# CDCgov/zoe

Measured on AMD Instinct MI355X. Metric: read-alignments/sec (150 bp vs 2 kb ref), higher is better.
Workload: dtype int16

## Files before the change

### include/zoe_sw.h

```cpp
#ifndef ZOE_SW_H
#define ZOE_SW_H

#include <stddef.h>
#include <stdint.h>

#ifdef __cplusplus
extern "C" {
#endif

typedef enum zsw_error {
    ZSW_OK = 0,
    ZSW_ERR_EMPTY_SEQUENCE = 1,
    ZSW_ERR_GAP_OPEN_OUT_OF_RANGE = 2,
    ZSW_ERR_GAP_EXTEND_OUT_OF_RANGE = 3,
    ZSW_ERR_BAD_GAP_WEIGHTS = 4,
    ZSW_ERR_INVALID_ARGUMENT = -1,
    ZSW_ERR_HIP = -2,
    ZSW_ERR_NO_DEVICE = -3,
    ZSW_ERR_UNSUPPORTED = -4,
    ZSW_ERR_NOT_CONFIGURED = -5
} zsw_error;

typedef enum zsw_status {
    ZSW_STATUS_SOME = 0,
// ... 291 lines not shown
    ZSW_DEBUG_NO_PIPELINE = 32,
    ZSW_DEBUG_ALIGN_NO_PACKED = 64,
    ZSW_DEBUG_SCORE_PRUNE = 128,
    ZSW_DEBUG_SCORE_PRUNE_ANY_SIZE = 256,
    ZSW_DEBUG_PRUNE_STRIP = 512,
    ZSW_DEBUG_ALIGN_LONG_WARMUP = 1024,
    ZSW_DEBUG_SEED_NO_BAND = 2048,
    ZSW_DEBUG_SEED_WIDE_BAND = 4096,
    ZSW_DEBUG_NO_ROW_CHUNKS = 8192,
    ZSW_DEBUG_RANGES_EXACT_REVERSE = 16384,
    ZSW_DEBUG_ALIGN_NO_CERTIFICATE = 32768,
    ZSW_DEBUG_SEED_STRIP_FIRST_TIER = 65536,
    ZSW_DEBUG_SEED_DIAG_LANE_EVENTS = 131072,
    ZSW_DEBUG_SEED_NO_COSCHEDULE = 262144,
    ZSW_DEBUG_SEED_PLAIN_KERNEL = 524288,
    ZSW_DEBUG_SEED_DIAG_MASKED = 1048576
} zsw_debug_flag;
zsw_error zsw_debug_set(zsw_context* ctx, uint32_t flags);

zsw_error zsw_debug_band_records(zsw_context* ctx, int32_t* records);

zsw_error zsw_debug_cert_records(zsw_context* ctx, int32_t* records);

zsw_error zsw_debug_threepass_records(zsw_context* ctx, int32_t* records);

zsw_error zsw_debug_strand_records(zsw_context* ctx, int32_t* records);

zsw_error zsw_debug_panel_records(zsw_context* ctx, int32_t* records);

typedef enum zsw_launch_kind {
    ZSW_LAUNCH_V1_FAST = 0,
// ... 25 lines not shown
```

### zoe_amd/_lib.py

```python
from __future__ import annotations

import ctypes as C
import os

_HERE = os.path.dirname(os.path.abspath(__file__))
LIB_PATH = os.path.join(_HERE, "libzoe_sw_hip.so")

ZSW_OK = 0
ERROR_NAMES = {
    0: "ZSW_OK",
    1: "ProfileError::EmptySequence",
    2: "ProfileError::GapOpenOutOfRange",
    3: "ProfileError::GapExtendOutOfRange",
    4: "ProfileError::BadGapWeights",
    -1: "ZSW_ERR_INVALID_ARGUMENT",
    -2: "ZSW_ERR_HIP",
    -3: "ZSW_ERR_NO_DEVICE",
    -4: "ZSW_ERR_UNSUPPORTED",
    -5: "ZSW_ERR_NOT_CONFIGURED",
}
MEM_HOST, MEM_DEVICE = 0, 1
DEBUG_SCORE_V1, DEBUG_NO_TILES, DEBUG_NO_W32, DEBUG_NO_WIDE, DEBUG_NO_SIDE_STREAMS, DEBUG_NO_PIPELINE, DEBUG_ALIGN_NO_PACKED = 1, 2, 4, 8, 16, 32, 64
DEBUG_SCORE_PRUNE, DEBUG_SCORE_PRUNE_ANY_SIZE, DEBUG_PRUNE_STRIP, DEBUG_ALIGN_LONG_WARMUP, DEBUG_SEED_NO_BAND, DEBUG_SEED_WIDE_BAND = 128, 256, 512, 1024, 2048, 4096
DEBUG_NO_ROW_CHUNKS = 8192
DEBUG_RANGES_EXACT_REVERSE = 16384
DEBUG_ALIGN_NO_CERTIFICATE = 32768
DEBUG_SEED_STRIP_FIRST_TIER = 65536
DEBUG_SEED_DIAG_LANE_EVENTS = 131072
DEBUG_SEED_NO_COSCHEDULE = 262144
DEBUG_SEED_PLAIN_KERNEL = 524288
DEBUG_SEED_DIAG_MASKED = 1048576
(LAUNCH_V1_FAST, LAUNCH_V1_BIASED, LAUNCH_V2, LAUNCH_WIDE, LAUNCH_V1_FAST_REV, LAUNCH_V1_BIASED_REV, LAUNCH_WIDE_REV, LAUNCH_TILE_V2, LAUNCH_TILE_WIDE,
 LAUNCH_TILE_W32, LAUNCH_EXACT32, LAUNCH_EXACT32_WORKLIST, LAUNCH_SEED_WINDOW, LAUNCH_SEED_BAND, LAUNCH_PRUNED, LAUNCH_ROW_CHUNKS) = range(16)
OPTION_EXACT_PRUNING = 1
OPTION_MIN_SCORE = 2
INT_TYPES = {"i8": 0, "i16": 1, "i32": 2, "u8": 3, "u16": 4, "u32": 5}

SYMBOLS = [
    "zsw_pack4_host", "zsw_create", "zsw_destroy", "zsw_last_error_string", "zsw_device_count", "zsw_set_scoring", "zsw_set_reference",
    "zsw_score_batch", "zsw_score_batch_from", "zsw_score_ends_batch", "zsw_score_ranges_batch", "zsw_score_ranges_batch_from", "zsw_align_batch", "zsw_align_batch_from", "zsw_align_3pass_batch", "zsw_align_3pass_batch_from", "zsw_sneaky_snake_batch",
    "zsw_set_profile_sequence", "zsw_score_shared_batch", "zsw_score_shared_batch_from", "zsw_score_ends_shared_batch", "zsw_score_ranges_shared_batch",
    "zsw_score_ranges_shared_batch_from", "zsw_align_shared_batch", "zsw_align_shared_batch_from", "zsw_align_3pass_shared_batch", "zsw_align_3pass_shared_batch_from",
    "zsw_synth_reads", "zsw_synth_reads_ragged", "zsw_synth_length", "zsw_synth_reference_host", "zsw_synth_reads_host",
    "zsw_synth_reads_ragged_host", "zsw_selftest", "zsw_timing_enable", "zsw_timing_read", "zsw_timing_read_window", "zsw_debug_set", "zsw_debug_band_records", "zsw_debug_cert_records", "zsw_debug_threepass_records", "zsw_prune_rescored", "zsw_set_option",
    "zsw_group_create", "zsw_group_destroy", "zsw_group_size", "zsw_group_context", "zsw_group_last_error_string", "zsw_group_set_scoring",
    "zsw_group_set_reference", "zsw_group_score_batch_from", "zsw_group_score_batch_from_device", "zsw_group_align_batch_from",
# ... 212 lines not shown
```

### zoe_amd/build.py

```python
from __future__ import annotations

import os
import shutil
import subprocess
import sys

HERE = os.path.dirname(os.path.abspath(__file__))
CSRC = os.path.join(HERE, "csrc")
LIB = os.path.join(HERE, "libzoe_sw_hip.so")
SOURCES = ["zsw_capi.hip", "zsw_capi_shared.hip", "zsw_shared.hip", "zsw_score.hip", "zsw_align.hip", "zsw_align_pk8.hip", "zsw_align_pk16.hip", "zsw_align_pk32.hip", "zsw_align_pk64.hip", "zsw_group.hip", "zsw_threepass.hip", "zsw_filter.hip", "zsw_score_wide.hip", "zsw_score_w32.hip", "zsw_score_prune.hip", "zsw_score_seed.hip", "zsw_score_seed_m0.hip", "zsw_score_seed_m1.hip", "zsw_score_seed_m2.hip", "zsw_score_band.hip", "zsw_multi.hip", "zsw_strand.hip", "zsw_panel.hip", "zsw_annotate.hip", "zsw_sam.hip", "zsw_pileup.hip", "zsw_text.hip", "zsw_fastq.hip", "zsw_samtext.hip", "zsw_fasta.hip"]
HEADERS = ["zsw_internal.hpp", "zsw_align_dev.hpp", "zsw_align_pk.hpp", "zsw_align_pk_kernel.hpp", "zsw_score_v1.hpp", "zsw_score_v2.hpp", "zsw_handback.hpp", "zsw_score_prune.hpp", "zsw_seed.hpp", "zsw_seed_packed.hpp", "zsw_seed_diag.hpp", "zsw_seed_diag_body.inc", "zsw_cert.hpp", "zsw_context.hpp", "zsw_shared.hpp", "zsw_score_seed.hpp", "zsw_score_seed_kernel.hpp", "zsw_align.hpp", "zsw_timer.hpp", "zsw_strand.hpp", "zsw_panel.hpp", "zsw_annotate.hpp", "zsw_sam.hpp", "zsw_pileup.hpp", "zsw_wave.hpp", "zsw_text.hpp", "zsw_text_dev.hpp", "zsw_fastq.hpp", "zsw_samtext.hpp", "zsw_fasta.hpp", "zsw_synth.h", "zsw_exports.map", os.path.join("..", "..", "include", "zoe_sw.h")]
ARCH = "gfx950"
EXTRA_FLAGS = {}


def _hipcc() -> str:
    for cand in (shutil.which("hipcc"), "/opt/rocm/bin/hipcc"):
        if cand and os.path.exists(cand):
            return cand
    raise RuntimeError("hipcc not found: the HIP extension cannot be built")


def needs_build() -> bool:
    if not os.path.exists(LIB):
        return True
# ... 75 lines not shown
```

### zoe_amd/csrc/zsw_capi.hip

```cpp
#include <map>
#include <new>
#include <utility>

#include "zsw_context.hpp"
#include "zsw_cert.hpp"
#include "zsw_strand.hpp"
#include "zsw_synth.h"

using namespace zsw;
using namespace zsw::capi;

namespace zsw {
namespace capi {


__global__ void maxlen_kernel(const uint64_t* offsets, uint32_t n, uint32_t* out) {
    uint32_t i = blockIdx.x * blockDim.x + threadIdx.x;
    uint32_t m = 0;
    for (; i < n; i += gridDim.x * blockDim.x) m = max(m, (uint32_t)(offsets[i + 1] - offsets[i]));
    for (int d = 32; d >= 1; d >>= 1) m = max(m, (uint32_t)__shfl_xor((int)m, d, 64));
    if ((threadIdx.x & 63) == 0) atomicMax(out, m);
}

__global__ void synth_kernel(uint64_t seed, uint64_t first, uint64_t n, uint32_t len, const uint8_t* ref, uint32_t R,
// ... 113 lines not shown
                           reads->offsets, n, ctx->d_maxlen.as<uint32_t>());
        uint32_t m = 0;
        ZSW_HIP(ctx, hipMemcpyAsync(&m, ctx->d_maxlen.p, 4, hipMemcpyDeviceToHost, stream));
        ZSW_HIP(ctx, hipStreamSynchronize(stream));
        st->max_len = m;
    }
    if (dest) st->dev = *dest;
    return ZSW_OK;
}

static zsw_error common_score_workspace(zsw_context* ctx, const Against& t, const zsw_batch* reads, hipStream_t stream, Staged* st) {
    const uint32_t n = st->b.n_reads;
    ZSW_HIP(ctx, ctx->d_fb_list.ensure((size_t)n * 4 + 4));
    ZSW_HIP(ctx, ctx->d_fb_count.ensure(4));
    if (reads->offsets || st->max_len > LONGEST_STRIP) ZSW_HIP(ctx, ctx->d_bucket_items.ensure((size_t)n * 4 + 4));
    if (reads->offsets && !ctx->side) {
        SideStreams* p = new (std::nothrow) SideStreams();
        if (p) {
            bool ok = hipEventCreateWithFlags(&p->fork, hipEventDisableTiming) == hipSuccess;
            for (int i = 0; ok && i < SideStreams::N; ++i)
                ok = hipStreamCreateWithFlags(&p->s[i], hipStreamNonBlocking) == hipSuccess &&
                     hipEventCreateWithFlags(&p->join[i], hipEventDisableTiming) == hipSuccess;
            if (ok) ctx->side = p;
            else delete p;
        }
    }
    if (st->max_len > LONGEST_STRIP) {
        const size_t per_pair = std::max<size_t>(t.len, 1) * 8, pairs = ((size_t)n + 1) / 2;
        const size_t want = 2 * std::min<size_t>(pairs * per_pair, std::max<size_t>(per_pair, size_t(512) << 20));
        ZSW_HIP(ctx, ctx->d_tile_buf.ensure(want));
        ZSW_HIP(ctx, ctx->d_tile_state.ensure((size_t)n * 16 + 16));
    }
    ZSW_HIP(ctx, ctx->d_bucket_counts.ensure(64 * 4));
    st->plan.min_counts = ctx->min_score != 0;
// ... 874 lines not shown
    for (DevBuf& b : ctx->sam_ws) b.release();
    for (DevBuf& b : ctx->pu_ws) b.release();
    for (DevBuf& b : ctx->text_ws) b.release();
    for (DevBuf& b : ctx->fq_ws) b.release();
    for (DevBuf& b : ctx->samtext_ws) b.release();
    seed_index_release(&ctx->seed);
    seed_index_release(&ctx->seed_rev);
    ctx->d_ref_rev.release();
    seed_index_release(&ctx->seed_shared);
    seed_index_release(&ctx->seed_shared_rev);
    panel_release(ctx);
    ctx->timer.destroy();
    ctx->timer_window.destroy();
    if (ctx->side) {
        (void)hipEventDestroy(ctx->side->fork);
        for (int i = 0; i < SideStreams::N; ++i) {
            (void)hipStreamDestroy(ctx->side->s[i]);
            (void)hipEventDestroy(ctx->side->join[i]);
        }
        delete ctx->side;
    }
    for (hipEvent_t ev : ctx->copy_events) (void)hipEventDestroy(ev);
    if (ctx->copy_stream) (void)hipStreamDestroy(ctx->copy_stream);
    delete ctx;
}

const char* zsw_last_error_string(const zsw_context* ctx) { return ctx ? ctx->err.c_str() : g_create_error.c_str(); }

zsw_error zsw_set_scoring(zsw_context* ctx, const int8_t* weights, int S, const uint8_t* index_map, int gap_open,
                          int gap_extend) {
// ... 358 lines not shown
```

### zoe_amd/csrc/zsw_handback.hpp

```cpp
#pragma once
#include <algorithm>
#include <cstdint>

namespace zsw {

struct StripCfg {
    int G, C;
};

inline bool strip_config_first_fit(const StripCfg* cfgs, int n_ascending, uint32_t max_len, int* G, int* C) {
    for (int k = 0; k < n_ascending; ++k) {
        if ((uint32_t)(cfgs[k].G * cfgs[k].C) >= max_len) {
            *G = cfgs[k].G;
            *C = cfgs[k].C;
            return true;
        }
    }
    return false;
}

inline bool strip_config_for_batch(const StripCfg* cfgs, int n_cfgs, uint32_t max_len, uint32_t n_items, int* G, int* C) {
    double best = 0;
    bool found = false;
    for (int k = 0; k < n_cfgs; ++k) {
// ... 59 lines not shown
struct CoscheduleRole {
    bool handback;
    uint32_t index;
};
constexpr CoscheduleRole coschedule_role(uint32_t block, uint32_t hb_blocks) {
    return block < hb_blocks ? CoscheduleRole{true, block} : CoscheduleRole{false, block - hb_blocks};
}
struct PairRange {
    uint32_t first, end;
};
constexpr PairRange handback_block_range(uint32_t block, int G, uint32_t count) {
    const uint64_t pairs = ((uint64_t)count + 1) / 2, lo = (uint64_t)block * handback_block_pairs(G), hi = lo + handback_block_pairs(G);
    return lo >= pairs ? PairRange{0u, 0u} : PairRange{(uint32_t)lo, (uint32_t)(hi < pairs ? hi : pairs)};
}

}
```

### zoe_amd/csrc/zsw_internal.hpp

```cpp
#pragma once
#include <hip/hip_runtime.h>
#include <stdint.h>

#include <string>
#include <vector>

#include "../../include/zoe_sw.h"

namespace zsw {

constexpr int MAX_S = 32;
constexpr uint32_t MIN2 = 0x80008000u;

struct ResultRule {
    uint64_t thr[3];
    uint8_t tier_code[3];
    int n_tiers;
};

__host__ __device__ inline void apply_rule(const ResultRule& r, uint64_t s, uint32_t* score, uint8_t* status,
                                           uint8_t* tier) {
    for (int k = 0; k < r.n_tiers; ++k) {
        if (s < r.thr[k]) {
            *score = (uint32_t)s;
// ... 33 lines not shown
    uint32_t* fb_list = nullptr;
    uint32_t* fb_count = nullptr;
    uint32_t* safe_row = nullptr;
    uint8_t* unique = nullptr;
    bool skip_handed_back = false;
    bool narrow_only = false;
    bool reads_reversed = false;
};

struct KernelTimer;

struct SideStreams {
    static constexpr int N = 8;
    hipStream_t s[N];
    hipEvent_t fork, join[N];
};

struct ScoreWorkspace {
    int32_t* scratch;
    size_t slots;
    uint32_t scratch_len;
    uint32_t* bucket_items;
    uint32_t* bucket_counts;
    uint2* tile_buf = nullptr;
    size_t tile_bytes = 0;
    uint4* tile_state = nullptr;
    SideStreams* side = nullptr;
    uint8_t* prune_work = nullptr;
    size_t prune_bytes = 0;
    uint32_t prune_chunk = 0;
// ... 39 lines not shown
```

### zoe_amd/csrc/zsw_score.hip

```cpp
#include <stdlib.h>

#include <algorithm>

#include "zsw_internal.hpp"
#include "zsw_score_v1.hpp"
#include "zsw_score_prune.hpp"
#include "zsw_score_seed.hpp"
#include "zsw_score_v2.hpp"
#include "zsw_handback.hpp"
#include "zsw_timer.hpp"

namespace zsw {

__global__ __launch_bounds__(64) void exact32_kernel(BatchDev b, const uint32_t* list, const uint32_t* list_count,
                                                     const uint8_t* ref, uint32_t ref_len, const ScoringDev* sc,
                                                     ResultRule rule, ScoreOut out, int32_t* scratch, uint32_t slots,
                                                     uint32_t scratch_len, const uint32_t* rev_ref_end,
                                                     const uint32_t* rev_query_end) {
    __shared__ uint8_t lut[256];
    __shared__ int32_t w[MAX_S * MAX_S];
    for (int i = threadIdx.x; i < 256; i += 64) lut[i] = sc->index_map[i];
    for (int i = threadIdx.x; i < MAX_S * MAX_S; i += 64) w[i] = sc->w[i];
    __syncthreads();
    const int S = sc->S;
// ... 188 lines not shown
        if (mode != 0 && out.ref_end) out.ref_end[id] = some ? row1 : 0;
        if (mode == 2 && out.query_end) out.query_end[id] = some ? col1 : 0;
    }
}

static hipError_t launch_table_cfg_v2(const ScoreArgsV2& a, int G, int C, int mode, hipStream_t stream) {
    switch (G * 100 + C) {
#define ZSW_CASE(GV, CV) \
    case GV * 100 + CV: return launch_cfg_v2<GV, CV>(a, mode, stream);
        ZSW_FOR_EACH_STRIP_CONFIG(ZSW_CASE)
#undef ZSW_CASE
    }
    return hipErrorInvalidValue;
}

static bool v2_ok(const ScoringDev& s, uint32_t debug) {
    if (debug & ZSW_DEBUG_SCORE_V1) return false;
    if (s.S > 7) return false;
    for (int r = 0; r < s.S; ++r)
        for (int q = 0; q < s.S; ++q) {
            const int t = s.w[r * s.S + q] + s.gap_extend;
            if (q < 4 ? (t < -128 || t > 127) : (t < 0 || t > 255)) return false;
        }
    return true;
}

static bool v2_range_setup(const ScoringDev& s, int G, ScoreArgsV2* a) {
    const int ge = s.gap_extend, go = s.gap_open;
    a->ge2 = (uint32_t)ge * 0x00010001u;
    a->gd2 = (uint32_t)(go - ge) * 0x00010001u;
// ... 344 lines not shown
            ah = tabs[t++];
            ah.b = ap.b;
            ah.n_items_dev = ap.n_items_dev;
            ah.first_item_dev = ap.first_item_dev;
        }
        ah.b.n_items = plan[k].grid_items;
        ah.gate_lo = plan[k].lo;
        ah.gate_hi = plan[k].hi;
        note_launch(c.ws.launch_log, ZSW_LAUNCH_V2, plan[k].G, plan[k].C, std::min(c.mode, 2));
        pe = launch_table_cfg_v2(ah, plan[k].G, plan[k].C, c.mode, stream);
    }
    return pe;
}

static hipError_t seed_items(ScoreDispatch& d, const BatchDev& bb, int g, int cc, uint32_t longest, size_t work_off, uint32_t list_off, uint32_t* counter,
                             uint32_t band_grid_cap, hipStream_t stream) {
    const ScoreCall& c = d.call;
    const ScoreWorkspace& ws = c.ws;
    if (!c.use_v2 || !ws.seed || !ws.seed_work || !ws.prune_fail_list || !(ws.debug & ZSW_DEBUG_SCORE_PRUNE) || (ws.debug & ZSW_DEBUG_PRUNE_STRIP))
        return hipErrorNotSupported;
    if (bb.n_items < SEED_MIN_READS && !(ws.debug & ZSW_DEBUG_SCORE_PRUNE_ANY_SIZE)) return hipErrorNotSupported;
    const size_t work_bytes = seed_workspace_bytes(bb.n_items, longest, band_grid_cap);
    if (g == 32 || work_off + work_bytes > ws.seed_bytes) return hipErrorNotSupported;
    ScoreArgsV2 ap = c.v2;
    if (!build_tables_v2(c.h_sc, g, &ap) || !seed_applicable(*ws.seed, longest, c.ref_len, ap.limit)) return hipErrorNotSupported;
    if (!ws.seed_gtab) return hipErrorNotSupported;
    ScoreArgsV2 ab = c.v2;
    const ScoreArgsV2* const band = !(ws.debug & ZSW_DEBUG_SEED_NO_BAND) && doubled_tables(c.h_sc, &ab) ? &ab : nullptr;
    hipError_t pe = build_seed_gtabs(d, ap, band, stream);
    if (pe != hipSuccess) return pe;
    pe = hipMemsetAsync(counter, 0, 4, stream);
    if (pe != hipSuccess) return pe;
    ap.b = bb;
    const RowChunks rc = row_chunks_for(c, longest);
    static_assert(2 + NCLS <= 32, "the n0 words sit 32 behind their counters");
    const SeedRegion region = {ws.seed_work + work_off, work_bytes, ws.prune_fail_list + list_off, counter, counter + 32};
    bool coscheduled = false;
    pe = launch_score_seeded(ap, g, cc, longest, ws, region, c.mode, band, band_grid_cap, rc.enabled, &coscheduled, stream);
    if (pe != hipSuccess) return pe;
    if (c.out.skip_handed_back) return hipSuccess;
    ap.b.items = region.fail_list;
    ap.n_items_dev = counter;
    ap.first_item_dev = coscheduled ? region.n0 : nullptr;
    pe = rc.enabled ? score_handed_back_chunked(c, ap, rc, g, cc, bb.n_items, stream) : score_handed_back_gated(c, ap, g, cc, longest, bb.n_items, stream);
    if (pe != hipSuccess) return pe;
    hipLaunchKernelGGL(add_count_kernel, dim3(1), dim3(1), 0, stream, counter, ws.prune_fail_count + 1);
    return hipGetLastError();
}

static hipError_t prune_items(const ScoreCall& c, const BatchDev& bb, int cls, uint32_t n_cls, hipStream_t stream) {
    const ScoreWorkspace& ws = c.ws;
    const bool wide = c.wide;
    if (!(c.use_v2 || wide) || !ws.prune_work || !(ws.debug & ZSW_DEBUG_SCORE_PRUNE)) return hipErrorNotSupported;
    if (!wide && !(ws.debug & ZSW_DEBUG_PRUNE_STRIP)) return hipErrorNotSupported;
    if (bb.n_items < PR_MIN_READS && !(ws.debug & ZSW_DEBUG_SCORE_PRUNE_ANY_SIZE)) return hipErrorNotSupported;
    const int last = n_cls < bb.n_items ? cls + 1 : cls;
    ScoreArgsV2 ap = c.v2;
    auto tables = [&](int g, ScoreArgsV2* t) { return wide ? build_tables_wide(c.h_sc, g, t) : build_tables_v2(c.h_sc, g, t); };
    if (!tables(1, &ap)) return hipErrorNotSupported;
    const uint32_t floor_strip = ap.floor0;
// ... 78 lines not shown
        for (int i = 0; i < SideStreams::N; ++i) {
            e = hipStreamWaitEvent(side->s[i], side->fork, 0);
            if (e != hipSuccess) return e;
        }
    }
    int used = 0;
    {
        size_t work_off = 0;
        uint32_t n_seedable = 0;
        for (int k = 0; k < NCLS; ++k) n_seedable += counts[k];
        for (int k = NCLS - 1; k >= 0; --k) {
            if (!counts[k]) continue;
            const Cfg& cf = kCfgs[kBucketCfg[k]];
            const uint32_t grid_cap = seed_band_class_cap(counts[k], n_seedable);
            e = seed_items(d, class_items(c, starts[k], counts[k]), cf.G, cf.C, caps.cap[k], work_off, starts[k], ws.prune_fail_count + 2 + k, grid_cap,
                           fork ? side->s[used % SideStreams::N] : stream);
            if (e == hipSuccess) {
                ++used;
                work_off += seed_workspace_bytes(counts[k], caps.cap[k], grid_cap);
                counts[k] = 0;
            } else if (e != hipErrorNotSupported) {
                return e;
            }
        }
    }
    {
        int k0[PR_N_CLASSES], k1[PR_N_CLASSES];
        uint32_t cnt[PR_N_CLASSES];
        for (int pc = 0; pc < PR_N_CLASSES; ++pc) {
            k0[pc] = k1[pc] = -1;
            cnt[pc] = 0;
// ... 65 lines not shown
        if (timer) timer->begin(stream);
        BatchDev bl = b;
        if (!bl.items && ws.bucket_items) {
            hipLaunchKernelGGL(iota_kernel, dim3((b.n_items + 255) / 256), dim3(256), 0, stream, ws.bucket_items, b.n_items);
            bl.items = ws.bucket_items;
        }
        e = launch_tiled(c, bl, max_len, stream);
        const bool tiled = e != hipErrorNotSupported;
        if (!tiled) e = launch_exact32(c, b, nullptr, nullptr, nullptr, nullptr, stream);
        if (timer) timer->end(stream);
        if (!tiled) return e;
    } else {
        if (timer) timer->begin(stream);
        e = hipErrorNotSupported;
        int Gs = 0, Cs = 0;
        if (score_config_for(max_len, &Gs, &Cs)) e = seed_items(d, b, Gs, Cs, max_len, 0, 0, ws.prune_fail_count, SEED_BAND_MAX_GRID, stream);
        const int cls = prune_class_for(max_len);
        if (e == hipErrorNotSupported && cls >= 0) e = prune_items(c, b, cls, b.n_items, stream);
        if (e == hipErrorNotSupported) e = launch_one(c, b, G, C, stream);
        if (timer) timer->end(stream);
    }
    if (e != hipSuccess) return e;
    return finish_worklist(c, stream);
}

hipError_t launch_score(const ScoringDev* d_sc, const ScoringDev& h_sc, const BatchDev& b, uint32_t max_len,
                        const uint8_t* d_ref, uint32_t ref_len, const ResultRule& rule, const ScoreOut& out,
                        const ScoreWorkspace& ws, hipStream_t stream, KernelTimer* timer, int mode) {
    hipError_t e = launch_score_passes(d_sc, h_sc, b, max_len, d_ref, ref_len, rule, out, ws, stream, timer, mode);
    if (e != hipSuccess || !ws.min_score || !ws.min_counts || b.n_items == 0) return e;
    hipLaunchKernelGGL(min_filter_kernel, dim3(std::min<uint32_t>((b.n_items + 255) / 256, 4096u)), dim3(256), 0, stream, b, min_threshold(rule, ws.min_score), out,
// ... 77 lines not shown
```

### zoe_amd/csrc/zsw_score_seed.hip

```cpp
#include <hipcub/hipcub.hpp>

#include <algorithm>
#include <vector>

#include "zsw_score_seed.hpp"
#include "zsw_seed_packed.hpp"
#include "zsw_score_v2.hpp"
#include "zsw_timer.hpp"

namespace zsw {

namespace {

struct SeedArgs {
    BatchDev b;
    const ScoringDev* sc;
    SeedParams sp;
    const uint2* table;
    uint32_t first, n;
    uint32_t* keys;
    uint32_t* ids;
    uint32_t* info;
    uint32_t* masks;
    uint32_t* band_masks;
// ... 238 lines not shown
    SeedParams p{};
    p.M1 = SEED_M1;
    p.M1_per8 = SEED_M1_PER8;
    p.Wd = SEED_WD;
    p.Wd_per16 = SEED_WD_PER16;
    return 7 * round256((size_t)n * 4 + 8) + round256((size_t)n + 8) + round256((size_t)n * seed_codes_stride(max_len) * 4 + 8) +
           round256(sort_temp_bytes(n)) + round256(seed_band_buffer_bytes(p, n, max_len, band_grid_cap)) + 256;
}

bool seed_applicable(const SeedIndex& ix, uint32_t max_len, uint32_t ref_len, uint32_t limit) {
    if (!ix.valid || !ix.usable || !ix.d_table || ref_len == 0 || ref_len >= (1u << 24)) return false;
    if (max_len < SEED_MIN_LEN || max_len > SEED_MAX_LEN) return false;
    return (uint64_t)ix.params.maxw * max_len + 8 < limit;
}

hipError_t launch_score_seeded(const ScoreArgsV2& a2, int G, int C, uint32_t max_len, const ScoreWorkspace& ws, const SeedRegion& r, int mode,
                               const ScoreArgsV2* band_tabs, uint32_t band_grid_cap, bool row_chunks, bool* coscheduled, hipStream_t stream) {
    const uint32_t n = a2.b.n_items;
    const SeedIndex& ix = *ws.seed;
    const uint32_t min_thr = (ws.min_score && ws.min_counts && !a2.out.skip_handed_back) ? min_threshold(a2.rule, ws.min_score) : 0u;
    const bool reads_reversed = a2.out.reads_reversed && a2.out.skip_handed_back;
    *coscheduled = false;
    if (n == 0) return hipSuccess;
    if (!r.work || !ws.seed_gtab || r.work_bytes < seed_workspace_bytes(n, max_len, band_grid_cap)) return hipErrorNotSupported;
    const bool band = band_tabs != nullptr && seed_band_applicable(ix.params, max_len, band_tabs->K, band_tabs->limit);
    const size_t per = round256((size_t)n * 4 + 8);
    uint32_t* keys = reinterpret_cast<uint32_t*>(r.work);
    uint32_t* keys_out = reinterpret_cast<uint32_t*>(r.work + per);
    uint32_t* ids = reinterpret_cast<uint32_t*>(r.work + 2 * per);
    uint32_t* order = reinterpret_cast<uint32_t*>(r.work + 3 * per);
    uint32_t* info = reinterpret_cast<uint32_t*>(r.work + 4 * per);
    uint32_t* masks = reinterpret_cast<uint32_t*>(r.work + 5 * per);
    uint32_t* band_masks = reinterpret_cast<uint32_t*>(r.work + 6 * per);
    uint8_t* p8 = r.work + 7 * per;
    uint8_t* band_dfb = p8;
    p8 += round256((size_t)n + 8);
    const uint32_t cs = seed_codes_stride(max_len);
    uint32_t* codes = reinterpret_cast<uint32_t*>(p8);
    p8 += round256((size_t)n * cs * 4 + 8);
    void* temp = p8;
// ... 28 lines not shown
    s.min_thr = min_thr;
    s.out = a2.out;
    s.min_count = ws.min_counts;
    const bool staged = !s.b.offsets && !s.b.items && s.b.fixed_len <= SEED_STAGE_LEN;
    const bool packed = staged && !(ws.debug & ZSW_DEBUG_SEED_PLAIN_KERNEL) && cs <= (uint32_t)SEED_PACKED_RES_WORDS_MAX;
    if (min_thr) {
        if (packed) hipLaunchKernelGGL((seed_packed_kernel<true>), dim3((n + 255) / 256), dim3(256), seed_packed_lds_bytes(s.b.fixed_len), stream, s);
        else if (staged) hipLaunchKernelGGL((seed_kernel<true, true>), dim3((n + 255) / 256), dim3(256), 0, stream, s);
        else hipLaunchKernelGGL((seed_kernel<false, true>), dim3((n + 255) / 256), dim3(256), 0, stream, s);
    } else if (packed)
        hipLaunchKernelGGL((seed_packed_kernel<false>), dim3((n + 255) / 256), dim3(256), seed_packed_lds_bytes(s.b.fixed_len), stream, s);
    else if (staged)
        hipLaunchKernelGGL((seed_kernel<true, false>), dim3((n + 255) / 256), dim3(256), 0, stream, s);
    else
        hipLaunchKernelGGL((seed_kernel<false, false>), dim3((n + 255) / 256), dim3(256), 0, stream, s);
    hipError_t e = hipcub::DeviceRadixSort::SortPairs(temp, temp_bytes, (const uint32_t*)keys, keys_out, (const uint32_t*)ids, order, (int)n, 0,
                                                      key_bits, stream);
    if (e != hipSuccess) return e;

    if (band) {
        SeedBandArgs b;
        b.b = a2.b;
        b.ref_len = a2.ref_len;
        b.ge2 = band_tabs->ge2;
        b.gd2 = band_tabs->gd2;
        b.floor0 = band_tabs->floor0;
        b.rule = a2.rule;
        b.out = a2.out;
        b.sp = ix.params;
        b.n = n;
        b.order = order;
// ... 17 lines not shown
        b.wd0 = ix.params.Wd;
        b.wd_per32 = 2 * ix.params.Wd_per16;
        b.n_dev = nullptr;
        b.retry = nullptr;
        b.min_thr = min_thr;
        b.min_count = ws.min_counts ? ws.min_counts + 1 : nullptr;
        uint32_t* queue1 = reinterpret_cast<uint32_t*>(r.work + 3 * per + (size_t)n * 4) + 1;
        uint32_t* queue2 = reinterpret_cast<uint32_t*>(r.work + (size_t)n * 4);
        e = hipMemsetAsync(queue1, 0, 4, stream);
        if (e != hipSuccess) return e;
        e = hipMemsetAsync(queue2, 0, 8, stream);
        if (e != hipSuccess) return e;
        uint32_t* accepted = queue2 + 1;
        b.next_pair = queue2;
        if (ws.window_timer) ws.window_timer->begin(stream);
        const uint32_t narrow_min_reads = (ws.debug & ZSW_DEBUG_SEED_WIDE_BAND) ? 0xffffffffu : (ws.debug & ZSW_DEBUG_SCORE_PRUNE_ANY_SIZE) ? 0u : SEED_NARROW_MIN_READS;
        if (max_len <= SEED_NARROW_MAX_LEN && n >= narrow_min_reads) {
            uint8_t* retry = reinterpret_cast<uint8_t*>(ids);
            uint32_t* order2 = keys_out;
            uint32_t* n2 = reinterpret_cast<uint32_t*>(r.work + 3 * per + (size_t)n * 4);
            e = hipMemsetAsync(retry, 0, n, stream);
            if (e != hipSuccess) return e;
            SeedBandArgs b1 = b;
            b1.wu0 = SEED_NARROW_WU;
            b1.wu_per16 = SEED_NARROW_WU_PER16;
            b1.wd0 = SEED_NARROW_WD;
            b1.wd_per32 = SEED_NARROW_WD_PER32;
            b1.retry = a2.out.narrow_only ? nullptr : retry;
            b1.accepted = a2.out.narrow_only ? nullptr : accepted;
            b1.next_pair = queue1;
            b1.diag_lane_events = (ws.debug & ZSW_DEBUG_SEED_DIAG_LANE_EVENTS) != 0;
            b1.diag_masked = (ws.debug & ZSW_DEBUG_SEED_DIAG_MASKED) != 0;
            note_launch(ws.launch_log, ZSW_LAUNCH_SEED_BAND, G, C, mode);
            const bool diagonal = mode == 0 && !a2.out.narrow_only && !(ws.debug & ZSW_DEBUG_SEED_STRIP_FIRST_TIER) && seed_diag_applicable(max_len, band_tabs->K);
            const CoscheduleCase cc{mode, !a2.out.narrow_only, diagonal, G, min_thr != 0, row_chunks, a2.out.skip_handed_back,
                                    (ws.debug & ZSW_DEBUG_SEED_NO_COSCHEDULE) != 0};
            if (handback_coschedule(cc)) {
                e = hipMemcpyAsync(r.n0, r.fail_count, 4, hipMemcpyDeviceToDevice, stream);
                if (e != hipSuccess) return e;
                ScoreArgsV2 hb = a2;
                hb.b.items = r.fail_list;
                hb.n_items_dev = r.fail_count;
                note_launch(ws.launch_log, ZSW_LAUNCH_V2, G, C, 0);
                e = launch_seed_diag_handback(b1, hb, G, C, stream);
                *coscheduled = true;
            } else {
                e = launch_seed_band(b1, mode, true, stream, diagonal);
            }
            if (e != hipSuccess) return e;
            if (a2.out.narrow_only) {
                if (ws.window_timer) ws.window_timer->end(stream);
                return hipSuccess;
            }
            e = hipcub::DeviceSelect::Flagged(temp, temp_bytes, (const uint32_t*)order, (const uint8_t*)retry, order2, n2, (int)n, stream);
            if (e != hipSuccess) return e;
            b.order = order2;
            b.n_dev = n2;
            b.wu0 = SEED_SECOND_WU;
            b.wu_per16 = SEED_SECOND_WU_PER16;
            b.wd0 = SEED_SECOND_WD;
// ... 103 lines not shown
```

### zoe_amd/csrc/zsw_score_seed.hpp

```cpp
#pragma once
#include "zsw_handback.hpp"
#include "zsw_internal.hpp"
#include "zsw_seed.hpp"

namespace zsw {

constexpr int SEED_M1 = 24;
constexpr int SEED_M1_PER8 = 1;
constexpr int SEED_M2 = 16;
constexpr int SEED_DN = 4;
constexpr int SEED_TOL = 8;
constexpr int SEED_DM = 4;
constexpr int SEED_WD = 9;
constexpr int SEED_WD_PER16 = 1;
constexpr int SEED_NARROW_WU = 8, SEED_NARROW_WU_PER16 = 0, SEED_NARROW_WD = 6, SEED_NARROW_WD_PER32 = 0;
constexpr uint32_t SEED_BAIL_RATIO = 40;
constexpr uint32_t SEED_BAIL_BELOW = 16384;
constexpr int SEED_SECOND_WU = 16, SEED_SECOND_WU_PER16 = 1, SEED_SECOND_WD = 8, SEED_SECOND_WD_PER32 = 1;
constexpr uint32_t SEED_NARROW_MAX_LEN = 640;
constexpr uint32_t SEED_NARROW_MIN_READS = 200000;
constexpr int SEED_BAND_SLACK = 32;
constexpr int SEED_DIAG_SLACK = 1;
constexpr uint32_t SEED_DIAG_MAX_LEN = 255;
constexpr uint32_t SEED_BAND_MAX_GRID = 1024;
// ... 82 lines not shown
constexpr uint32_t SEED_BAND_CLASS_MIN_GRID = 64;
inline uint32_t seed_band_class_cap(uint32_t n_class, uint32_t n_total) {
    return SEED_BAND_CLASS_MIN_GRID + (uint32_t)((uint64_t)SEED_BAND_MAX_GRID * n_class / (n_total ? n_total : 1));
}
size_t seed_workspace_bytes(uint32_t n, uint32_t max_len, uint32_t band_grid_cap = SEED_BAND_MAX_GRID);
bool seed_applicable(const SeedIndex& ix, uint32_t max_len, uint32_t ref_len, uint32_t limit);
hipError_t seed_build_gtab(const ScoreArgsV2& a2, uint2* gtab, hipStream_t stream);
inline uint2* seed_gtab_band(const ScoreWorkspace& ws, uint32_t ref_len) { return ws.seed_gtab + (ref_len + 2 * SEED_GTAB_PAD); }
struct SeedRegion {
    uint8_t* work;
    size_t work_bytes;
    uint32_t* fail_list;
    uint32_t* fail_count;
    uint32_t* n0;
};
hipError_t launch_score_seeded(const ScoreArgsV2& a2, int G, int C, uint32_t max_len, const ScoreWorkspace& ws, const SeedRegion& r, int mode,
                               const ScoreArgsV2* band_tabs, uint32_t band_grid_cap, bool row_chunks, bool* coscheduled, hipStream_t stream);
hipError_t seed_index_update(SeedIndex* ix, const ScoringDev& sc, const uint8_t* h_ref, size_t ref_len);
void seed_index_release(SeedIndex* ix);

hipError_t launch_seed_window_m0(const SeedWindowArgs& a, int G, int C, hipStream_t stream);
hipError_t launch_seed_window_m1(const SeedWindowArgs& a, int G, int C, hipStream_t stream);
hipError_t launch_seed_window_m2(const SeedWindowArgs& a, int G, int C, hipStream_t stream);

}
```

Measured before the change: 787.3 million.

## Split handed-back reads into slices scored concurrently on side streams

Splits the list of reads handed back by the seed filter into a shared slice, an optional head slice and a tail slice. A tiny device kernel computes the slice bounds, and the tail slice is scored on a side stream with a narrower G=8 config that fits in registers beside the band kernel. Ordering between streams uses events. This aims to overlap full-DP rescoring of failed reads with the seed band pass and fill idle SIMDs. In exchange it adds cross-stream events, creates side streams for large non-ragged batches, and risks contention with the co-scheduled band kernel.

```diff
diff --git a/include/zoe_sw.h b/include/zoe_sw.h
--- a/include/zoe_sw.h
+++ b/include/zoe_sw.h
@@ -329,7 +329,9 @@
     ZSW_DEBUG_SEED_DIAG_LANE_EVENTS = 131072,
     ZSW_DEBUG_SEED_NO_COSCHEDULE = 262144,
     ZSW_DEBUG_SEED_PLAIN_KERNEL = 524288,
-    ZSW_DEBUG_SEED_DIAG_MASKED = 1048576
+    ZSW_DEBUG_SEED_DIAG_MASKED = 1048576,
+    ZSW_DEBUG_SEED_NO_SLICES = 2097152,
+    ZSW_DEBUG_SEED_TINY_SLICES = 4194304
 } zsw_debug_flag;
 zsw_error zsw_debug_set(zsw_context* ctx, uint32_t flags);
 
diff --git a/zoe_amd/_lib.py b/zoe_amd/_lib.py
--- a/zoe_amd/_lib.py
+++ b/zoe_amd/_lib.py
@@ -30,6 +30,8 @@
 DEBUG_SEED_NO_COSCHEDULE = 262144
 DEBUG_SEED_PLAIN_KERNEL = 524288
 DEBUG_SEED_DIAG_MASKED = 1048576
+DEBUG_SEED_NO_SLICES = 2097152
+DEBUG_SEED_TINY_SLICES = 4194304
 (LAUNCH_V1_FAST, LAUNCH_V1_BIASED, LAUNCH_V2, LAUNCH_WIDE, LAUNCH_V1_FAST_REV, LAUNCH_V1_BIASED_REV, LAUNCH_WIDE_REV, LAUNCH_TILE_V2, LAUNCH_TILE_WIDE,
  LAUNCH_TILE_W32, LAUNCH_EXACT32, LAUNCH_EXACT32_WORKLIST, LAUNCH_SEED_WINDOW, LAUNCH_SEED_BAND, LAUNCH_PRUNED, LAUNCH_ROW_CHUNKS) = range(16)
 OPTION_EXACT_PRUNING = 1
diff --git a/zoe_amd/build.py b/zoe_amd/build.py
--- a/zoe_amd/build.py
+++ b/zoe_amd/build.py
@@ -8,7 +8,7 @@
 HERE = os.path.dirname(os.path.abspath(__file__))
 CSRC = os.path.join(HERE, "csrc")
 LIB = os.path.join(HERE, "libzoe_sw_hip.so")
-SOURCES = ["zsw_capi.hip", "zsw_capi_shared.hip", "zsw_shared.hip", "zsw_score.hip", "zsw_align.hip", "zsw_align_pk8.hip", "zsw_align_pk16.hip", "zsw_align_pk32.hip", "zsw_align_pk64.hip", "zsw_group.hip", "zsw_threepass.hip", "zsw_filter.hip", "zsw_score_wide.hip", "zsw_score_w32.hip", "zsw_score_prune.hip", "zsw_score_seed.hip", "zsw_score_seed_m0.hip", "zsw_score_seed_m1.hip", "zsw_score_seed_m2.hip", "zsw_score_band.hip", "zsw_multi.hip", "zsw_strand.hip", "zsw_panel.hip", "zsw_annotate.hip", "zsw_sam.hip", "zsw_pileup.hip", "zsw_text.hip", "zsw_fastq.hip", "zsw_samtext.hip", "zsw_fasta.hip"]
+SOURCES = ["zsw_capi.hip", "zsw_capi_shared.hip", "zsw_shared.hip", "zsw_score.hip", "zsw_align.hip", "zsw_align_pk8.hip", "zsw_align_pk16.hip", "zsw_align_pk32.hip", "zsw_align_pk64.hip", "zsw_group.hip", "zsw_threepass.hip", "zsw_filter.hip", "zsw_score_wide.hip", "zsw_score_w32.hip", "zsw_score_prune.hip", "zsw_score_seed.hip", "zsw_score_seed_m0.hip", "zsw_score_seed_m1.hip", "zsw_score_seed_m2.hip", "zsw_score_band.hip", "zsw_handback_split.hip", "zsw_multi.hip", "zsw_strand.hip", "zsw_panel.hip", "zsw_annotate.hip", "zsw_sam.hip", "zsw_pileup.hip", "zsw_text.hip", "zsw_fastq.hip", "zsw_samtext.hip", "zsw_fasta.hip"]
 HEADERS = ["zsw_internal.hpp", "zsw_align_dev.hpp", "zsw_align_pk.hpp", "zsw_align_pk_kernel.hpp", "zsw_score_v1.hpp", "zsw_score_v2.hpp", "zsw_handback.hpp", "zsw_score_prune.hpp", "zsw_seed.hpp", "zsw_seed_packed.hpp", "zsw_seed_diag.hpp", "zsw_seed_diag_body.inc", "zsw_cert.hpp", "zsw_context.hpp", "zsw_shared.hpp", "zsw_score_seed.hpp", "zsw_score_seed_kernel.hpp", "zsw_align.hpp", "zsw_timer.hpp", "zsw_strand.hpp", "zsw_panel.hpp", "zsw_annotate.hpp", "zsw_sam.hpp", "zsw_pileup.hpp", "zsw_wave.hpp", "zsw_text.hpp", "zsw_text_dev.hpp", "zsw_fastq.hpp", "zsw_samtext.hpp", "zsw_fasta.hpp", "zsw_synth.h", "zsw_exports.map", os.path.join("..", "..", "include", "zoe_sw.h")]
 ARCH = "gfx950"
 EXTRA_FLAGS = {}
diff --git a/zoe_amd/csrc/zsw_capi.hip b/zoe_amd/csrc/zsw_capi.hip
--- a/zoe_amd/csrc/zsw_capi.hip
+++ b/zoe_amd/csrc/zsw_capi.hip
@@ -151,10 +151,13 @@
     ZSW_HIP(ctx, ctx->d_fb_list.ensure((size_t)n * 4 + 4));
     ZSW_HIP(ctx, ctx->d_fb_count.ensure(4));
     if (reads->offsets || st->max_len > LONGEST_STRIP) ZSW_HIP(ctx, ctx->d_bucket_items.ensure((size_t)n * 4 + 4));
-    if (reads->offsets && !ctx->side) {
+    const bool slices = !reads->offsets && !(ctx->flags() & ZSW_DEBUG_SEED_NO_SLICES) && (n >= HANDBACK_SLICE_MIN_CLASS || (ctx->flags() & ZSW_DEBUG_SEED_TINY_SLICES));
+    if ((reads->offsets || slices) && !ctx->side) {
         SideStreams* p = new (std::nothrow) SideStreams();
         if (p) {
-            bool ok = hipEventCreateWithFlags(&p->fork, hipEventDisableTiming) == hipSuccess;
+            bool ok = hipEventCreateWithFlags(&p->fork, hipEventDisableTiming) == hipSuccess &&
+                      hipEventCreateWithFlags(&p->seeded, hipEventDisableTiming) == hipSuccess &&
+                      hipEventCreateWithFlags(&p->shared, hipEventDisableTiming) == hipSuccess;
             for (int i = 0; ok && i < SideStreams::N; ++i)
                 ok = hipStreamCreateWithFlags(&p->s[i], hipStreamNonBlocking) == hipSuccess &&
                      hipEventCreateWithFlags(&p->join[i], hipEventDisableTiming) == hipSuccess;
@@ -1059,6 +1062,8 @@
     ctx->timer_window.destroy();
     if (ctx->side) {
         (void)hipEventDestroy(ctx->side->fork);
+        (void)hipEventDestroy(ctx->side->seeded);
+        (void)hipEventDestroy(ctx->side->shared);
         for (int i = 0; i < SideStreams::N; ++i) {
             (void)hipStreamDestroy(ctx->side->s[i]);
             (void)hipEventDestroy(ctx->side->join[i]);
diff --git a/zoe_amd/csrc/zsw_handback.hpp b/zoe_amd/csrc/zsw_handback.hpp
--- a/zoe_amd/csrc/zsw_handback.hpp
+++ b/zoe_amd/csrc/zsw_handback.hpp
@@ -97,4 +97,53 @@
     return lo >= pairs ? PairRange{0u, 0u} : PairRange{(uint32_t)lo, (uint32_t)(hi < pairs ? hi : pairs)};
 }
 
+constexpr uint32_t HANDBACK_SIMDS = 1024;
+constexpr uint32_t HANDBACK_VGPRS_PER_SIMD = 512;
+constexpr uint32_t HANDBACK_VGPRS_BAND = 256;
+constexpr uint32_t HANDBACK_VGPRS_REMAINDER = 48;
+constexpr int HANDBACK_TAIL_G = 8;
+constexpr uint32_t HANDBACK_VGPRS_TAIL = HANDBACK_TAIL_G == 4 ? 144 : 96;
+constexpr uint32_t HANDBACK_TAIL_WAVES_PER_SIMD = (HANDBACK_VGPRS_PER_SIMD - HANDBACK_VGPRS_BAND - HANDBACK_VGPRS_REMAINDER) / HANDBACK_VGPRS_TAIL;
+static_assert(HANDBACK_TAIL_G == 4 || HANDBACK_TAIL_G == 8, "the register counts above are those of <4,38> and <8,19>");
+static_assert(HANDBACK_TAIL_WAVES_PER_SIMD >= 1 &&
+                  HANDBACK_TAIL_WAVES_PER_SIMD * HANDBACK_VGPRS_TAIL + HANDBACK_VGPRS_BAND + HANDBACK_VGPRS_REMAINDER <= HANDBACK_VGPRS_PER_SIMD,
+              "the second tier's blocks must find registers beside the tail slice");
+constexpr uint32_t HANDBACK_WAVE_READS = 2 * 64 / 4;
+constexpr uint32_t HANDBACK_TAIL_MAX_READS = HANDBACK_TAIL_WAVES_PER_SIMD * HANDBACK_SIMDS * (2 * 64 / HANDBACK_TAIL_G);
+constexpr uint32_t HANDBACK_TAIL_READS = HANDBACK_SIMDS * (2 * 64 / HANDBACK_TAIL_G);
+static_assert(HANDBACK_TAIL_READS <= HANDBACK_TAIL_MAX_READS, "the tail's bound from the register file");
+constexpr uint32_t HANDBACK_HEAD_READS = 0;
+constexpr uint32_t HANDBACK_ROUND_READS = 3 * HANDBACK_SIMDS * HANDBACK_WAVE_READS;
+constexpr uint32_t HANDBACK_SLICE_MIN_CLASS = 1u << 21;
+constexpr uint32_t HANDBACK_TINY_TAIL_READS = 128, HANDBACK_TINY_HEAD_READS = 128, HANDBACK_TINY_HEAD_MIN = 1;
+
+struct ItemRange {
+    uint32_t first, end;
+};
+struct HandbackSlices {
+    ItemRange shared, head, tail;
+};
+struct HandbackSliceRule {
+    uint32_t keep;
+    uint32_t tail_reads, tail_min;
+    uint32_t head_reads, head_min;
+    constexpr bool head() const { return head_reads != 0; }
+    constexpr bool tail() const { return tail_reads != 0; }
+};
+constexpr HandbackSliceRule handback_slice_rule(bool coscheduled, bool own_stream, uint32_t class_reads, bool no_slices, bool tiny) {
+    if (!coscheduled || !own_stream || no_slices) return HandbackSliceRule{0u, 0u, 0u, 0u, 0u};
+    if (tiny) return HandbackSliceRule{0u, HANDBACK_TINY_TAIL_READS, HANDBACK_TINY_TAIL_READS, HANDBACK_TINY_HEAD_READS, HANDBACK_TINY_HEAD_MIN};
+    if (class_reads < HANDBACK_SLICE_MIN_CLASS) return HandbackSliceRule{0u, 0u, 0u, 0u, 0u};
+    return HandbackSliceRule{HANDBACK_ROUND_READS, HANDBACK_TAIL_READS, HANDBACK_TAIL_READS, HANDBACK_HEAD_READS, HANDBACK_HEAD_READS};
 }
+constexpr HandbackSlices handback_slices(uint32_t n0, const HandbackSliceRule& r) {
+    uint32_t avail = n0 > r.keep ? n0 - r.keep : 0u;
+    const uint32_t tail = (r.tail_reads && avail >= r.tail_min) ? (avail < r.tail_reads ? avail : r.tail_reads) : 0u;
+    avail -= tail;
+    const uint32_t head = (r.head_reads && avail >= r.head_min) ? (avail < r.head_reads ? avail : r.head_reads) : 0u;
+    const uint32_t s = n0 - tail - head;
+    return HandbackSlices{{0u, s}, {s, s + head}, {s + head, n0}};
+}
+constexpr int HANDBACK_BOUND_WORDS = 2;
+
+}
diff --git a/zoe_amd/csrc/zsw_handback_split.hip b/zoe_amd/csrc/zsw_handback_split.hip
--- /dev/null
+++ b/zoe_amd/csrc/zsw_handback_split.hip
@@ -0,0 +1,27 @@
+#include <hip/hip_runtime.h>
+
+#include "zsw_handback.hpp"
+#include "zsw_score_seed.hpp"
+
+namespace zsw {
+
+namespace {
+
+__global__ void handback_split_kernel(const uint32_t* count, uint32_t* n0, uint32_t* bounds, HandbackSliceRule rule) {
+    const uint32_t n = *count;
+    *n0 = n;
+    if (bounds) {
+        const HandbackSlices s = handback_slices(n, rule);
+        bounds[0] = s.shared.end;
+        bounds[1] = s.head.end;
+    }
+}
+
+}
+
+hipError_t launch_handback_split(const uint32_t* count, uint32_t* n0, uint32_t* bounds, const HandbackSliceRule& rule, hipStream_t stream) {
+    hipLaunchKernelGGL(handback_split_kernel, dim3(1), dim3(1), 0, stream, count, n0, bounds, rule);
+    return hipGetLastError();
+}
+
+}
diff --git a/zoe_amd/csrc/zsw_internal.hpp b/zoe_amd/csrc/zsw_internal.hpp
--- a/zoe_amd/csrc/zsw_internal.hpp
+++ b/zoe_amd/csrc/zsw_internal.hpp
@@ -71,6 +71,7 @@
     static constexpr int N = 8;
     hipStream_t s[N];
     hipEvent_t fork, join[N];
+    hipEvent_t seeded, shared;
 };
 
 struct ScoreWorkspace {
diff --git a/zoe_amd/csrc/zsw_score.hip b/zoe_amd/csrc/zsw_score.hip
--- a/zoe_amd/csrc/zsw_score.hip
+++ b/zoe_amd/csrc/zsw_score.hip
@@ -226,6 +226,8 @@
     return hipErrorInvalidValue;
 }
 
+hipError_t launch_score_v2_cfg(const ScoreArgsV2& a, int G, int C, int mode, hipStream_t stream) { return launch_table_cfg_v2(a, G, C, mode, stream); }
+
 static bool v2_ok(const ScoringDev& s, uint32_t debug) {
     if (debug & ZSW_DEBUG_SCORE_V1) return false;
     if (s.S > 7) return false;
@@ -600,7 +602,7 @@
 }
 
 static hipError_t seed_items(ScoreDispatch& d, const BatchDev& bb, int g, int cc, uint32_t longest, size_t work_off, uint32_t list_off, uint32_t* counter,
-                             uint32_t band_grid_cap, hipStream_t stream) {
+                             uint32_t band_grid_cap, const SideStreams* slice_streams, hipStream_t stream) {
     const ScoreCall& c = d.call;
     const ScoreWorkspace& ws = c.ws;
     if (!c.use_v2 || !ws.seed || !ws.seed_work || !ws.prune_fail_list || !(ws.debug & ZSW_DEBUG_SCORE_PRUNE) || (ws.debug & ZSW_DEBUG_PRUNE_STRIP))
@@ -620,9 +622,32 @@
     ap.b = bb;
     const RowChunks rc = row_chunks_for(c, longest);
     static_assert(2 + NCLS <= 32, "the n0 words sit 32 behind their counters");
+    static_assert(2 + NCLS <= 32 - HANDBACK_BOUND_WORDS, "the slice bounds take the last words behind the n0 words");
     const SeedRegion region = {ws.seed_work + work_off, work_bytes, ws.prune_fail_list + list_off, counter, counter + 32};
+    HandbackSliceLaunch sl{};
+    sl.rule = handback_slice_rule(true, slice_streams != nullptr && counter == ws.prune_fail_count, bb.n_items, (ws.debug & ZSW_DEBUG_SEED_NO_SLICES) != 0,
+                                  (ws.debug & ZSW_DEBUG_SEED_TINY_SLICES) != 0);
+    const bool slices = sl.rule.head() || sl.rule.tail();
+    ScoreArgsV2 tail_tabs = c.v2;
+    if (slices) {
+        sl.bounds = ws.prune_fail_count + 64 - HANDBACK_BOUND_WORDS;
+        sl.head = slice_streams->s[0];
+        sl.tail = slice_streams->s[1];
+        sl.seeded = slice_streams->seeded;
+        sl.shared = slice_streams->shared;
+        sl.tail_tabs = &ap;
+        sl.tail_G = g;
+        sl.tail_C = cc;
+        for (int k = 0; k < N_ASCENDING_CFGS && HANDBACK_TAIL_G != g && sl.tail_G == g; ++k) {
+            if (kCfgs[k].G != HANDBACK_TAIL_G || (uint32_t)(kCfgs[k].G * kCfgs[k].C) < longest || !build_tables_v2(c.h_sc, kCfgs[k].G, &tail_tabs)) continue;
+            tail_tabs.b = bb;
+            sl.tail_tabs = &tail_tabs;
+            sl.tail_G = kCfgs[k].G;
+            sl.tail_C = kCfgs[k].C;
+        }
+    }
     bool coscheduled = false;
-    pe = launch_score_seeded(ap, g, cc, longest, ws, region, c.mode, band, band_grid_cap, rc.enabled, &coscheduled, stream);
+    pe = launch_score_seeded(ap, g, cc, longest, ws, region, c.mode, band, band_grid_cap, rc.enabled, &coscheduled, slices ? &sl : nullptr, stream);
     if (pe != hipSuccess) return pe;
     if (c.out.skip_handed_back) return hipSuccess;
     ap.b.items = region.fail_list;
@@ -630,6 +655,14 @@
     ap.first_item_dev = coscheduled ? region.n0 : nullptr;
     pe = rc.enabled ? score_handed_back_chunked(c, ap, rc, g, cc, bb.n_items, stream) : score_handed_back_gated(c, ap, g, cc, longest, bb.n_items, stream);
     if (pe != hipSuccess) return pe;
+    if (coscheduled && slices) {
+        for (int i = 0; i < 2; ++i) {
+            if (!(i == 0 ? sl.rule.head() : sl.rule.tail())) continue;
+            pe = hipEventRecord(slice_streams->join[i], slice_streams->s[i]);
+            if (pe == hipSuccess) pe = hipStreamWaitEvent(stream, slice_streams->join[i], 0);
+            if (pe != hipSuccess) return pe;
+        }
+    }
     hipLaunchKernelGGL(add_count_kernel, dim3(1), dim3(1), 0, stream, counter, ws.prune_fail_count + 1);
     return hipGetLastError();
 }
@@ -738,7 +771,7 @@
             const Cfg& cf = kCfgs[kBucketCfg[k]];
             const uint32_t grid_cap = seed_band_class_cap(counts[k], n_seedable);
             e = seed_items(d, class_items(c, starts[k], counts[k]), cf.G, cf.C, caps.cap[k], work_off, starts[k], ws.prune_fail_count + 2 + k, grid_cap,
-                           fork ? side->s[used % SideStreams::N] : stream);
+                           nullptr, fork ? side->s[used % SideStreams::N] : stream);
             if (e == hipSuccess) {
                 ++used;
                 work_off += seed_workspace_bytes(counts[k], caps.cap[k], grid_cap);
@@ -834,7 +867,7 @@
         if (timer) timer->begin(stream);
         e = hipErrorNotSupported;
         int Gs = 0, Cs = 0;
-        if (score_config_for(max_len, &Gs, &Cs)) e = seed_items(d, b, Gs, Cs, max_len, 0, 0, ws.prune_fail_count, SEED_BAND_MAX_GRID, stream);
+        if (score_config_for(max_len, &Gs, &Cs)) e = seed_items(d, b, Gs, Cs, max_len, 0, 0, ws.prune_fail_count, SEED_BAND_MAX_GRID, ws.side, stream);
         const int cls = prune_class_for(max_len);
         if (e == hipErrorNotSupported && cls >= 0) e = prune_items(c, b, cls, b.n_items, stream);
         if (e == hipErrorNotSupported) e = launch_one(c, b, G, C, stream);
diff --git a/zoe_amd/csrc/zsw_score_seed.hip b/zoe_amd/csrc/zsw_score_seed.hip
--- a/zoe_amd/csrc/zsw_score_seed.hip
+++ b/zoe_amd/csrc/zsw_score_seed.hip
@@ -276,8 +276,24 @@
     return (uint64_t)ix.params.maxw * max_len + 8 < limit;
 }
 
+static hipError_t launch_handback_slice(ScoreArgsV2 a, int G, int C, const uint32_t* list, const uint32_t* first, const uint32_t* end, uint32_t most,
+                                        hipEvent_t after, hipStream_t from, hipStream_t side, std::vector<uint32_t>* launch_log) {
+    hipError_t e = hipEventRecord(after, from);
+    if (e == hipSuccess) e = hipStreamWaitEvent(side, after, 0);
+    if (e != hipSuccess) return e;
+    a.b.items = list;
+    a.b.n_items = most;
+    a.n_items_dev = end;
+    a.first_item_dev = first;
+    a.gate_lo = 0;
+    a.gate_hi = 0xffffffffu;
+    note_launch(launch_log, ZSW_LAUNCH_V2, G, C, 0);
+    return launch_score_v2_cfg(a, G, C, 0, side);
+}
+
 hipError_t launch_score_seeded(const ScoreArgsV2& a2, int G, int C, uint32_t max_len, const ScoreWorkspace& ws, const SeedRegion& r, int mode,
-                               const ScoreArgsV2* band_tabs, uint32_t band_grid_cap, bool row_chunks, bool* coscheduled, hipStream_t stream) {
+                               const ScoreArgsV2* band_tabs, uint32_t band_grid_cap, bool row_chunks, bool* coscheduled, const HandbackSliceLaunch* slices,
+                               hipStream_t stream) {
     const uint32_t n = a2.b.n_items;
     const SeedIndex& ix = *ws.seed;
     const uint32_t min_thr = (ws.min_score && ws.min_counts && !a2.out.skip_handed_back) ? min_threshold(a2.rule, ws.min_score) : 0u;
@@ -286,6 +302,14 @@
     if (n == 0) return hipSuccess;
     if (!r.work || !ws.seed_gtab || r.work_bytes < seed_workspace_bytes(n, max_len, band_grid_cap)) return hipErrorNotSupported;
     const bool band = band_tabs != nullptr && seed_band_applicable(ix.params, max_len, band_tabs->K, band_tabs->limit);
+    const uint32_t narrow_min_reads = (ws.debug & ZSW_DEBUG_SEED_WIDE_BAND) ? 0xffffffffu : (ws.debug & ZSW_DEBUG_SCORE_PRUNE_ANY_SIZE) ? 0u : SEED_NARROW_MIN_READS;
+    const bool two_tiers = band && max_len <= SEED_NARROW_MAX_LEN && n >= narrow_min_reads;
+    const bool diagonal = two_tiers && mode == 0 && !a2.out.narrow_only && !(ws.debug & ZSW_DEBUG_SEED_STRIP_FIRST_TIER) && seed_diag_applicable(max_len, band_tabs->K);
+    const CoscheduleCase cc{mode, two_tiers && !a2.out.narrow_only, diagonal, G, min_thr != 0, row_chunks, a2.out.skip_handed_back,
+                            (ws.debug & ZSW_DEBUG_SEED_NO_COSCHEDULE) != 0};
+    const bool cosched = handback_coschedule(cc);
+    const HandbackSliceRule slice_rule = cosched && slices ? slices->rule : HandbackSliceRule{0u, 0u, 0u, 0u, 0u};
+    const bool sliced = slice_rule.head() || slice_rule.tail();
     const size_t per = round256((size_t)n * 4 + 8);
     uint32_t* keys = reinterpret_cast<uint32_t*>(r.work);
     uint32_t* keys_out = reinterpret_cast<uint32_t*>(r.work + per);
@@ -344,7 +368,15 @@
         hipLaunchKernelGGL((seed_kernel<true, false>), dim3((n + 255) / 256), dim3(256), 0, stream, s);
     else
         hipLaunchKernelGGL((seed_kernel<false, false>), dim3((n + 255) / 256), dim3(256), 0, stream, s);
-    hipError_t e = hipcub::DeviceRadixSort::SortPairs(temp, temp_bytes, (const uint32_t*)keys, keys_out, (const uint32_t*)ids, order, (int)n, 0,
+    hipError_t e = hipSuccess;
+    if (cosched) {
+        e = launch_handback_split(r.fail_count, r.n0, sliced ? slices->bounds : nullptr, slice_rule, stream);
+        if (e == hipSuccess && slice_rule.head())
+            e = launch_handback_slice(a2, G, C, r.fail_list, slices->bounds, slices->bounds + 1, slice_rule.head_reads, slices->seeded, stream, slices->head,
+                                      ws.launch_log);
+        if (e != hipSuccess) return e;
+    }
+    e = hipcub::DeviceRadixSort::SortPairs(temp, temp_bytes, (const uint32_t*)keys, keys_out, (const uint32_t*)ids, order, (int)n, 0,
                                                       key_bits, stream);
     if (e != hipSuccess) return e;
 
@@ -392,8 +424,7 @@
         uint32_t* accepted = queue2 + 1;
         b.next_pair = queue2;
         if (ws.window_timer) ws.window_timer->begin(stream);
-        const uint32_t narrow_min_reads = (ws.debug & ZSW_DEBUG_SEED_WIDE_BAND) ? 0xffffffffu : (ws.debug & ZSW_DEBUG_SCORE_PRUNE_ANY_SIZE) ? 0u : SEED_NARROW_MIN_READS;
-        if (max_len <= SEED_NARROW_MAX_LEN && n >= narrow_min_reads) {
+        if (two_tiers) {
             uint8_t* retry = reinterpret_cast<uint8_t*>(ids);
             uint32_t* order2 = keys_out;
             uint32_t* n2 = reinterpret_cast<uint32_t*>(r.work + 3 * per + (size_t)n * 4);
@@ -410,18 +441,16 @@
             b1.diag_lane_events = (ws.debug & ZSW_DEBUG_SEED_DIAG_LANE_EVENTS) != 0;
             b1.diag_masked = (ws.debug & ZSW_DEBUG_SEED_DIAG_MASKED) != 0;
             note_launch(ws.launch_log, ZSW_LAUNCH_SEED_BAND, G, C, mode);
-            const bool diagonal = mode == 0 && !a2.out.narrow_only && !(ws.debug & ZSW_DEBUG_SEED_STRIP_FIRST_TIER) && seed_diag_applicable(max_len, band_tabs->K);
-            const CoscheduleCase cc{mode, !a2.out.narrow_only, diagonal, G, min_thr != 0, row_chunks, a2.out.skip_handed_back,
-                                    (ws.debug & ZSW_DEBUG_SEED_NO_COSCHEDULE) != 0};
-            if (handback_coschedule(cc)) {
-                e = hipMemcpyAsync(r.n0, r.fail_count, 4, hipMemcpyDeviceToDevice, stream);
-                if (e != hipSuccess) return e;
+            if (cosched) {
                 ScoreArgsV2 hb = a2;
                 hb.b.items = r.fail_list;
-                hb.n_items_dev = r.fail_count;
+                hb.n_items_dev = sliced ? slices->bounds : r.fail_count;
                 note_launch(ws.launch_log, ZSW_LAUNCH_V2, G, C, 0);
                 e = launch_seed_diag_handback(b1, hb, G, C, stream);
                 *coscheduled = true;
+                if (e == hipSuccess && slice_rule.tail())
+                    e = launch_handback_slice(*slices->tail_tabs, slices->tail_G, slices->tail_C, r.fail_list, slices->bounds + 1, r.n0, slice_rule.tail_reads,
+                                              slices->shared, stream, slices->tail, ws.launch_log);
             } else {
                 e = launch_seed_band(b1, mode, true, stream, diagonal);
             }
diff --git a/zoe_amd/csrc/zsw_score_seed.hpp b/zoe_amd/csrc/zsw_score_seed.hpp
--- a/zoe_amd/csrc/zsw_score_seed.hpp
+++ b/zoe_amd/csrc/zsw_score_seed.hpp
@@ -120,8 +120,19 @@
     uint32_t* fail_count;
     uint32_t* n0;
 };
+struct HandbackSliceLaunch {
+    HandbackSliceRule rule;
+    uint32_t* bounds;
+    hipStream_t head, tail;
+    hipEvent_t seeded, shared;
+    const ScoreArgsV2* tail_tabs;
+    int tail_G, tail_C;
+};
 hipError_t launch_score_seeded(const ScoreArgsV2& a2, int G, int C, uint32_t max_len, const ScoreWorkspace& ws, const SeedRegion& r, int mode,
-                               const ScoreArgsV2* band_tabs, uint32_t band_grid_cap, bool row_chunks, bool* coscheduled, hipStream_t stream);
+                               const ScoreArgsV2* band_tabs, uint32_t band_grid_cap, bool row_chunks, bool* coscheduled, const HandbackSliceLaunch* slices,
+                               hipStream_t stream);
+hipError_t launch_handback_split(const uint32_t* count, uint32_t* n0, uint32_t* bounds, const HandbackSliceRule& rule, hipStream_t stream);
+hipError_t launch_score_v2_cfg(const ScoreArgsV2& a, int G, int C, int mode, hipStream_t stream);
 hipError_t seed_index_update(SeedIndex* ix, const ScoringDev& sc, const uint8_t* h_ref, size_t ref_len);
 void seed_index_release(SeedIndex* ix);
 
```

After: 801.9 million (median of 6 runs). 1.9% higher.
